# ethz-asl/voxgraph

Hardware: AMD Instinct MI355X
Metric: Mresiduals+Jacobians/s per GPU; full pose-graph solve ms (200 submaps) (higher is better)
Workload: dtype f32

## Files before the change

### voxgraph_amd/csrc/vgx_internal.h

```cpp
#ifndef VGX_INTERNAL_H_
#define VGX_INTERNAL_H_

#include <hip/hip_runtime.h>

#include <algorithm>
#include <atomic>
#include <cstdint>
#include <mutex>
#include <condition_variable>
#include <initializer_list>
#include <random>
#include <string>
#include <utility>
#include <vector>

#include "voxgraph_amd.h"

namespace vgx {


template <int VPS, int LAYOUT>
struct BrickLayout {
  static constexpr int B = VPS + 1;
  static constexpr int S = VPS / 4;
// ... 40 lines not shown
  float cos_emo, sin_emo;
  float dxs, dxc;
  float dys, dyc;
  float k1, k2;
  float pad;
};
static_assert(sizeof(PosePack) == 64, "PosePack must stay one 64-byte line");

struct alignas(16) ConstraintDev {
  GridDev grid;
  const float4* xyzd;
  const float* weight;
  const uint32_t* sample_raw;
  const double* cumulative;
  const int32_t* search_lut;
  int32_t search_buckets;
  const float4* sample_pts;
  const int32_t* inv_order;
  int64_t n_points;
  const float4* chunk_bounds;
  int64_t n;
  int64_t row0;
  int64_t prow0;
  int32_t tile_points;
  double factor;
  double no_corr_cost;
};

struct Tile {
  int32_t constraint;
  int32_t count;
  int64_t start;
};

constexpr int kMinSearchBuckets = 4096;
constexpr int kMaxSearchBuckets = 1 << 24;
constexpr int kChunkPoints = 512;
constexpr int kNormalSize = 45;
constexpr int kPartialSize = 22;

struct Context {
  int device = 0;
  hipStream_t own_stream = nullptr;
  hipStream_t stream = nullptr;
  hipEvent_t ev_start = nullptr, ev_stop = nullptr;
  std::mutex mu;
  hipStream_t tsdf_own_stream = nullptr;
  hipStream_t tsdf_stream = nullptr;
  bool stream_priorities = false;
  std::atomic<int> tsdf_integrators{0};
  hipEvent_t ev_tsdf_start = nullptr, ev_tsdf_stop = nullptr, ev_handover = nullptr;
  std::mutex tsdf_mu;
  std::mutex err_mu;
  std::string last_error;
  int cu_count = 256;
  int brick_layout = 0;
  int sampling_bricks = 1;
  struct EvalSlot {
    hipStream_t stream = nullptr;
    hipEvent_t order = nullptr;
    double* d_out = nullptr;
    int64_t out_rows = 0;
    uint32_t* d_raw = nullptr;
    uint32_t* h_raw = nullptr;
    int64_t raw_cap = 0;
    double* h_out = nullptr;
// ... 108 lines not shown
  uint32_t* d_sample_raw = nullptr;
  uint32_t* h_sample_raw = nullptr;
  std::mutex mu;
  int draw_raw(uint32_t* out);
  vgx::SamplerEngine& engine();
  bool sampling() const { return cfg.sampling_ratio != -1.0f; }
  bool points_current() const;
  vgx::ConstraintDev describe() const;
  int users = 0;
  bool destroy_requested = false;
};

struct vgx_reg_batch_s {
  vgx_ctx ctx = nullptr;
  int32_t n = 0;
  int32_t n_global = 0;
  int layout = 0;
  std::vector<vgx_reg> regs;
  std::vector<int32_t> node_pair;
  std::vector<int32_t> global_index;
  std::vector<int64_t> row_offset;
  std::vector<vgx::Tile> tiles;
  vgx::ConstraintDev* d_desc = nullptr;
  vgx::PosePack* d_pack = nullptr;
  vgx::PosePack* h_pack = nullptr;
  hipEvent_t pack_copied[2] = {nullptr, nullptr};
  int pack_turn = 0;
  vgx::Tile* d_tiles = nullptr;
  vgx::Tile* d_draw_tiles = nullptr;
  int32_t n_draw_tiles = 0;
  float4* d_drawn = nullptr;
  int32_t* d_drawn_idx = nullptr;
  unsigned char* d_tile_dead = nullptr;
  int32_t* d_tile_first = nullptr;
  double* d_partials = nullptr;
  double* d_normal = nullptr;
  double* h_normal = nullptr;
  int32_t* d_node_pair = nullptr;
  int32_t* d_global_index = nullptr;
  std::vector<vgx::Tile> reduce_tiles;
  std::vector<vgx::ConstraintDev> host_desc;
  std::vector<int32_t> host_tile_first;
  bool launch_order_made = false;
  bool launch_order_grouped = false, points_order_grouped = false;
  bool points_order_made = false;
  std::vector<int32_t> host_points_tile_first;
  vgx::Tile* d_reduce_tiles = nullptr;
  int32_t csr_nodes = 0;
  int32_t* d_node_first = nullptr;
  int32_t* d_node_items = nullptr;
  struct StreamJob {
    vgx::SamplerEngine* engine;
    int64_t offset;
    int64_t count;
  };
  std::vector<StreamJob> stream_jobs;
  uint32_t* d_raw = nullptr;
  void* d_stream_jobs = nullptr;
  bool any_sampling = false;
  bool holds_regs = false;
  double* d_rows[3] = {nullptr, nullptr, nullptr};
  char* h_rows = nullptr;
  bool rows_have[3] = {false, false, false};
  bool rows_mirrored = false;
};

namespace vgx {
#ifndef VGX_TOOLING_LIBRARY
int set_error(vgx_ctx ctx, int code, const std::string& msg);
#else
inline int set_error(vgx_ctx ctx, int code, const std::string& msg);
#endif

std::mutex& lifetime_mu();

struct DeviceBuffer {
  void* p = nullptr;
  size_t bytes = 0;
// ... 139 lines not shown
```

### voxgraph_amd/csrc/vgx_reg.hip

```cpp
#include <algorithm>
#include <cmath>
#include <cstdio>
#include <cstdlib>
#include <cstring>
#include <numeric>

#include "vgx_internal.h"

#pragma clang fp contract(off)

namespace vgx {

namespace {
struct YawQuat {
  float w, z;
};

YawQuat yaw_exp(float psi) {
  float nrm = std::sqrt(0.0f * 0.0f + 0.0f * 0.0f + psi * psi);
  double theta = (double)nrm;
  double na = theta < std::pow(2.220446049250313e-16, 0.25)
                  ? 0.5 + (theta * theta) * (1.0 / 48.0)
                  : std::sin(theta * 0.5) / theta;
  double ct = std::cos(theta * 0.5);
// ... 365 lines not shown
  }
}

__device__ __forceinline__ f32x4 sampled_point(const ConstraintDev& C, int64_t i) {
  if (C.sample_pts) return as_global(reinterpret_cast<const f32x4*>(C.sample_pts))[C.row0 + i];
  return as_global(reinterpret_cast<const f32x4*>(C.xyzd))[weighted_draw(C, i)];
}


__device__ __forceinline__ bool tile_cullable(const ConstraintDev& C) {
  return C.no_corr_cost == 0.0 && C.sample_raw == nullptr && C.chunk_bounds != nullptr;
}
template <int PPT>
__device__ __forceinline__ bool tile_outside(const ConstraintDev& C, const PosePack& P, const Tile& tile) {
  const long long chunk0 = tile.start / kChunkPoints;
  bool any_live = false;
#pragma unroll
  for (int q = 0; q < (kBlockThreads * PPT) / kChunkPoints; ++q)
    if (q * kChunkPoints < tile.count) any_live |= !chunk_outside(C.grid, P, C.chunk_bounds[chunk0 + q]);
  return !any_live;
}
template <int PPT>
__global__ __launch_bounds__(256) void reg_points_tile_dead_kernel(const ConstraintDev* __restrict__ cons,
                                                                  const PosePack* __restrict__ packs,
                                                                  const Tile* __restrict__ tiles, int n_tiles,
                                                                  unsigned char* __restrict__ dead) {
  const int t = blockIdx.x * 256 + threadIdx.x;
  if (t >= n_tiles) return;
  const Tile tile = tiles[t];
  const ConstraintDev& C = cons[tile.constraint];
  dead[t] = tile_cullable(C) && tile_outside<PPT>(C, packs[tile.constraint], tile);
}

template <int VPS, int LAYOUT, typename OUT, int PPT>
__device__ __forceinline__ void reg_eval_points_body(
    const ConstraintDev& C, const PosePack& P, const Tile& tile, int dead_hint, OUT* __restrict__ residuals,
    typename Out4<OUT>::type* __restrict__ jac_ref, typename Out4<OUT>::type* __restrict__ jac_read) {
  const GridDev g = C.grid;
  const bool sampled = C.sample_raw != nullptr;
  const bool want_jac = (jac_ref != nullptr) | (jac_read != nullptr);
  {
    bool any_live = dead_hint == 0;
    if (dead_hint < 0) {
      any_live = true;
      if (tile_cullable(C)) any_live = !tile_outside<PPT>(C, P, tile);
    }
    if (!any_live) {
#pragma unroll
      for (int j = 0; j < PPT; ++j) {
        int local = j * kBlockThreads + (int)threadIdx.x;
        if (local >= tile.count) continue;
        int64_t row = C.row0 + tile.start + local;
        store_out(&residuals[row], (OUT)0);
        if (jac_ref) store_out4(&jac_ref[row], Out4<OUT>::make(0.0, 0.0, 0.0, 0.0));
        if (jac_read) store_out4(&jac_read[row], Out4<OUT>::make(0.0, 0.0, 0.0, 0.0));
      }
      return;
    }
  }

  f32x4 pt[PPT];
  float w[PPT];
  const float* cell[PPT];
  float Dx[PPT], Dy[PPT], Dz[PPT];
  float d[PPT][8];
#pragma unroll
  for (int j = 0; j < PPT; ++j) {
    int local = j * kBlockThreads + (int)threadIdx.x;
    bool active = local < tile.count;
    int64_t i = tile.start + (active ? local : 0);
    if (sampled) {
      pt[j] = sampled_point(C, i);
      w[j] = 1.0f;
    } else {
      pt[j] = as_global(reinterpret_cast<const f32x4*>(C.xyzd))[i];
      w[j] = as_global(C.weight)[i];
    }
  }
  Located loc[PPT];
  bool have[PPT];
  const bool grid_empty = g.bricks == nullptr;
#pragma unroll
  for (int j = 0; j < PPT; ++j) {
    loc[j] = locate_stage1<VPS, LAYOUT>(g, P, pt[j].x, pt[j].y, pt[j].z);
    Dx[j] = loc[j].Dx;
    Dy[j] = loc[j].Dy;
    Dz[j] = loc[j].Dz;
    have[j] = false;
#pragma unroll
    for (int k = 0; k < 8; ++k) d[j][k] = 0.0f;
    cell[j] = nullptr;
  }
  if (!grid_empty) {
    int slot[PPT];
#pragma unroll
    for (int j = 0; j < PPT; ++j) slot[j] = as_global(g.lut)[loc[j].lut_index];
    constexpr int CELLS = BrickLayout<VPS, LAYOUT>::cells;
#pragma unroll
    for (int j = 0; j < PPT; ++j) {
      have[j] = loc[j].inside && slot[j] >= 0;
      cell[j] = g.bricks + (size_t)(have[j] ? slot[j] : 0) * CELLS + loc[j].cell_off;
    }
#pragma unroll
    for (int j = 0; j < PPT; ++j) load_neighbours<VPS, LAYOUT>(cell[j], d[j]);
  }
#pragma unroll
  for (int j = 0; j < PPT; ++j) {
    int local = j * kBlockThreads + (int)threadIdx.x;
    if (local >= tile.count) continue;
    PointEval e = eval_point(d[j], have[j], Dx[j], Dy[j], Dz[j], g.voxel_size_inv, P,
                             pt[j].x, pt[j].y, pt[j].w, w[j], C.no_corr_cost, want_jac);
    int64_t row = C.row0 + tile.start + local;
    const double f = C.factor;
    store_out(&residuals[row], (OUT)(e.r * f));
    if (jac_ref)
      store_out4(&jac_ref[row], Out4<OUT>::make((double)e.jo0 * f, (double)e.jo1 * f,
                                                (double)e.jo2 * f, (double)e.jo3 * f));
    if (jac_read)
      store_out4(&jac_read[row], Out4<OUT>::make((double)-e.jo0 * f, (double)-e.jo1 * f,
                                                 (double)-e.jo2 * f, (double)e.je3 * f));
  }
}

template <int VPS, int LAYOUT, typename OUT, int PPT>
__global__ __launch_bounds__(kBlockThreads) void reg_eval_points_kernel(
    const ConstraintDev* __restrict__ cons, const PosePack* __restrict__ packs,
    const Tile* __restrict__ tiles, const unsigned char* __restrict__ tile_dead, int n_tiles,
    OUT* __restrict__ residuals, typename Out4<OUT>::type* __restrict__ jac_ref,
    typename Out4<OUT>::type* __restrict__ jac_read, int blocked) {
  const int t = blockIdx.x;
  if (t >= n_tiles) return;
  const Tile tile = tiles[t];
  const int dead = tile_dead[t];
  const ConstraintDev& C = cons[tile.constraint];
  if (blocked) {
    using O4 = typename Out4<OUT>::type;
    constexpr long long kBlockBytes = (long long)(PPT * kBlockThreads) * (long long)(sizeof(OUT) + 2 * sizeof(O4));
    const long long first = C.row0 + tile.start;
    char* blk = reinterpret_cast<char*>(residuals) + ((C.prow0 + tile.start) / (PPT * kBlockThreads)) * kBlockBytes;
    OUT* r_t = reinterpret_cast<OUT*>(blk) - first;
    O4* jr_t = reinterpret_cast<O4*>(blk + (long long)(PPT * kBlockThreads) * (long long)sizeof(OUT)) - first;
    O4* je_t = reinterpret_cast<O4*>(blk + (long long)(PPT * kBlockThreads) * (long long)(sizeof(OUT) + sizeof(O4))) - first;
    reg_eval_points_body<VPS, LAYOUT, OUT, PPT>(C, packs[tile.constraint], tile, dead, r_t, jr_t, je_t);
    return;
  }
  reg_eval_points_body<VPS, LAYOUT, OUT, PPT>(C, packs[tile.constraint], tile, dead, residuals, jac_ref, jac_read);
}

template <int VPS, int LAYOUT, typename OUT, int PPT>
__global__ __launch_bounds__(kBlockThreads) void reg_eval_points_single_kernel(
    ConstraintDev C, PosePack P, int n_tiles, OUT* __restrict__ residuals,
    typename Out4<OUT>::type* __restrict__ jac_ref, typename Out4<OUT>::type* __restrict__ jac_read) {
  const int t = blockIdx.x;
  if (t >= n_tiles) return;
  Tile tile;
  tile.constraint = 0;
  tile.start = (int64_t)t * (kBlockThreads * PPT);
  int64_t left = C.n - tile.start;
  tile.count = (int32_t)(left < kBlockThreads * PPT ? left : kBlockThreads * PPT);
  reg_eval_points_body<VPS, LAYOUT, OUT, PPT>(C, P, tile, -1, residuals, jac_ref, jac_read);
}

constexpr int kReduceIters = 10;
constexpr int kLeanPointsPerThread = 2;
constexpr int kLeanWaves = 6;
constexpr bool kBallotSkip = true;

__device__ __forceinline__ bool eval_point_lean(const float c[8], bool have, float Dx, float Dy, float Dz,
                                                float value, float inv_f, const PosePack& P, float xi, float yi,
                                                float d_ref, float w, float u[6]) {
#pragma clang fp contract(fast)
  const float q4 = Dx * Dy, q5 = Dy * Dz, q6 = Dz * Dx;
  const float gx = q5 * c[7] + (Dz * c[6] + (Dy * c[4] + c[1]));
  const float gy = q6 * c[7] + (Dz * c[5] + (Dx * c[4] + c[2]));
  const float gz = q4 * c[7] + (Dx * c[6] + (Dy * c[5] + c[3]));
  const float val = value;
  const bool ok = have && (val == val);
  const float s = -w * inv_f;
  const float h0 = ok ? s * gx : 0.0f, h1 = ok ? s * gy : 0.0f, h2 = ok ? s * gz : 0.0f;
// ... 363 lines not shown
          }
        }
      }
      out.push_back(stream[(size_t)src][next[(size_t)src]++]);
    }
  return out;
}

static std::vector<Tile> make_draw_order(const std::vector<ConstraintDev>& desc,
                                         const std::vector<int32_t>& tile_first, const std::vector<Tile>& tiles) {
  std::vector<const void*> key;
  std::vector<std::vector<Tile>> group_tiles;
  std::vector<int64_t> group_work;
  size_t n = 0;
  for (size_t c = 0; c < desc.size(); ++c) {
    if (!desc[c].sample_raw) continue;
    size_t g = 0;
    while (g < key.size() && key[g] != (const void*)desc[c].cumulative) ++g;
    if (g == key.size()) {
      key.push_back((const void*)desc[c].cumulative);
      group_tiles.emplace_back();
      group_work.push_back(0);
    }
    for (int32_t t = tile_first[c]; t < tile_first[c + 1]; ++t) {
      group_tiles[g].push_back(tiles[(size_t)t]);
      group_work[g] += tiles[(size_t)t].count;
      ++n;
    }
  }
  return deal_to_xcds(group_tiles, group_work, n);
}

static bool make_xcd_order(const std::vector<ConstraintDev>& desc, const std::vector<int32_t>& tile_first,
                           const std::vector<int32_t>& tile_work, std::vector<Tile>& tiles, bool points_pass) {
  if (points_pass) {
    const char* e = getenv("VGX_POINTS_TILE_ORDER");
    if (e && atoi(e) == 0) return false;
  }
  const int n = (int)desc.size();
  if (n < 2 || tiles.size() < 16) return false;
  std::vector<std::vector<int>> groups;
  {
    std::vector<std::pair<const void*, int>> key;
    for (int c = 0; c < n; ++c) {
      int g = -1;
      if (!desc[(size_t)c].sample_raw)
        for (auto& k : key)
          if (k.first == (const void*)desc[(size_t)c].xyzd) g = k.second;
      if (g < 0) {
        g = (int)groups.size();
        groups.emplace_back();
        if (!desc[(size_t)c].sample_raw) key.emplace_back((const void*)desc[(size_t)c].xyzd, g);
      }
      groups[(size_t)g].push_back(c);
    }
  }
  std::vector<std::vector<Tile>> group_tiles(groups.size());
  std::vector<int64_t> group_work(groups.size(), 0);
  for (size_t g = 0; g < groups.size(); ++g) {
    int most = 0;
    for (int c : groups[g]) most = std::max(most, tile_first[(size_t)c + 1] - tile_first[(size_t)c]);
    for (int r = 0; r < most; ++r)
      for (int c : groups[g])
        if (r < tile_first[(size_t)c + 1] - tile_first[(size_t)c]) {
          const size_t t = (size_t)tile_first[(size_t)c] + (size_t)r;
          group_tiles[g].push_back(tiles[t]);
          group_work[g] += points_pass ? (int64_t)tiles[t].count * 36 + (int64_t)tile_work[t] * 52
                                       : (int64_t)tile_work[t] + 256;
        }
  }
  constexpr double kOrderShareMin = 0.3;
  constexpr double kOrderLiveMin = 0.75;
  {
    int64_t total = 0, shareable = 0;
    for (size_t g = 0; g < groups.size(); ++g) {
      int most = 0;
      for (int c : groups[g]) most = std::max(most, tile_first[(size_t)c + 1] - tile_first[(size_t)c]);
      for (int r = 0; r < most; ++r) {
        int64_t sum = 0, mx = 0;
        for (int c : groups[g])
          if (r < tile_first[(size_t)c + 1] - tile_first[(size_t)c]) {
            const int64_t w = tile_work[(size_t)tile_first[(size_t)c] + (size_t)r];
            sum += w;
            mx = std::max(mx, w);
          }
        total += sum;
        shareable += sum - mx;
      }
    }
    if (total == 0 || (double)shareable < kOrderShareMin * (double)total) return false;
    int64_t all_points = 0;
    for (const Tile& t : tiles) all_points += t.count;
    if ((double)total < kOrderLiveMin * (double)all_points) return false;
  }
  std::vector<Tile> out = deal_to_xcds(group_tiles, group_work, tiles.size());
  tiles.swap(out);
  return true;
}

__global__ __launch_bounds__(256) void reg_finalize_kernel(const ConstraintDev* __restrict__ cons,
                                                          const PosePack* __restrict__ packs,
// ... 133 lines not shown
      int item = node_items[it];
      int c = item >> 1, side = item & 1;
      const double* nb = normal + (size_t)c * kNormalSize;
      if (e < 4) {
        v += nb[1 + 4 * side + e];
      } else {
        int k = (e - 4) / 4, l = (e - 4) % 4;
        v += H(nb, 4 * side + k, 4 * side + l);
      }
    }
    double* dst = e < 4 ? &fused[1 + 4 * (int64_t)node + e]
                        : &fused[1 + 4 * (int64_t)n_nodes + 16 * (int64_t)node + (e - 4)];
    *dst = accumulate ? *dst + v : v;
  } else if (tid < n_node_elems + n_off) {
    int64_t o = tid - n_node_elems;
    int c = (int)(o / 16), e = (int)(o % 16);
    const double* nb = normal + (size_t)c * kNormalSize;
    int gidx = global_index[c];
    double* dst = &fused[1 + 20 * (int64_t)n_nodes + 16 * (int64_t)gidx + e];
    double v = H(nb, e / 4, 4 + e % 4);
    *dst = accumulate ? *dst + v : v;
  }
}

__global__ void reg_scatter_normal_kernel(const double* __restrict__ normal, int n, const int32_t* __restrict__ global_index,
                                          double* __restrict__ all) {
  const int64_t tid = (int64_t)blockIdx.x * blockDim.x + threadIdx.x;
  if (tid >= (int64_t)n * kNormalSize) return;
  const int c = (int)(tid / kNormalSize), e = (int)(tid % kNormalSize);
  all[(size_t)global_index[c] * kNormalSize + e] = normal[tid];
}

template <typename OUT>
static void launch_points(vgx_ctx ctx, int vps, int layout, const ConstraintDev* d_desc, const PosePack* d_pack,
                          const Tile* d_tiles, unsigned char* d_tile_dead, int n_tiles, void* res, void* jr,
                          void* je, bool blocked = false) {
  if (n_tiles <= 0) return;
  hipLaunchKernelGGL(reg_points_tile_dead_kernel<kPointsPerThread>, dim3((n_tiles + 255) / 256), dim3(256), 0,
                     ctx->stream, d_desc, d_pack, d_tiles, n_tiles, d_tile_dead);
  dim3 grid(((n_tiles + 7) / 8) * 8), block(kBlockThreads);
  using O4 = typename Out4<OUT>::type;
#define VGX_LAUNCH_POINTS(VPS, LAYOUT)                                                              \
  hipLaunchKernelGGL((reg_eval_points_kernel<VPS, LAYOUT, OUT, kPointsPerThread>), grid, block, 0, \
                     ctx->stream, d_desc, d_pack, d_tiles, d_tile_dead, n_tiles, (OUT*)res, (O4*)jr, (O4*)je, blocked ? 1 : 0)
  if (layout == 0) {
    if (vps == 16) VGX_LAUNCH_POINTS(16, 0);
    else VGX_LAUNCH_POINTS(8, 0);
  } else if (layout == 1) {
    if (vps == 16) VGX_LAUNCH_POINTS(16, 1);
    else VGX_LAUNCH_POINTS(8, 1);
  } else {
    if (vps == 16) VGX_LAUNCH_POINTS(16, 2);
    else VGX_LAUNCH_POINTS(8, 2);
  }
#undef VGX_LAUNCH_POINTS
}

template <typename OUT>
static void launch_points_single(hipStream_t stream, int vps, const ConstraintDev& desc, const PosePack& pack,
                                 void* res, void* jr, void* je) {
  const int n_tiles = (int)((desc.n + kTilePoints - 1) / kTilePoints);
  if (n_tiles <= 0) return;
  dim3 grid(((n_tiles + 7) / 8) * 8), block(kBlockThreads);
  using O4 = typename Out4<OUT>::type;
#define VGX_LAUNCH_SINGLE(VPS, LAYOUT)                                                                       \
  hipLaunchKernelGGL((reg_eval_points_single_kernel<VPS, LAYOUT, OUT, kPointsPerThread>), grid, block, 0, stream, \
                     desc, pack, n_tiles, (OUT*)res, (O4*)jr, (O4*)je)
  const int layout = desc.grid.layout;
  if (layout == 0) {
    if (vps == 16) VGX_LAUNCH_SINGLE(16, 0);
    else VGX_LAUNCH_SINGLE(8, 0);
  } else if (layout == 1) {
    if (vps == 16) VGX_LAUNCH_SINGLE(16, 1);
    else VGX_LAUNCH_SINGLE(8, 1);
  } else {
    if (vps == 16) VGX_LAUNCH_SINGLE(16, 2);
    else VGX_LAUNCH_SINGLE(8, 2);
// ... 555 lines not shown
    b->holds_regs = true;
  }
  *out = b;
  return VGX_OK;
}

int vgx_reg_batch_destroy(vgx_reg_batch b) {
  if (!b) return VGX_ERR_INVALID;
  (void)hipSetDevice(b->ctx->device);
  (void)hipStreamSynchronize(b->ctx->stream);
  std::vector<vgx_reg> orphans;
  if (b->holds_regs) {
    std::lock_guard<std::mutex> lt(lifetime_mu());
    for (vgx_reg r : b->regs)
      if (--r->users == 0 && r->destroy_requested) orphans.push_back(r);
  }
  for (vgx_reg r : orphans) (void)vgx_reg_destroy(r);
  for (int a = 0; a < 3; ++a)
    if (b->d_rows[a]) (void)hipFree(b->d_rows[a]);
  if (b->h_rows) (void)hipHostFree(b->h_rows);
  if (b->d_raw) (void)hipFree(b->d_raw);
  if (b->d_stream_jobs) (void)hipFree(b->d_stream_jobs);
  if (b->d_node_first) (void)hipFree(b->d_node_first);
  if (b->d_node_items) (void)hipFree(b->d_node_items);
  if (b->d_reduce_tiles) (void)hipFree(b->d_reduce_tiles);
  if (b->d_desc) (void)hipFree(b->d_desc);
  if (b->d_pack) (void)hipFree(b->d_pack);
  if (b->h_pack) (void)hipHostFree(b->h_pack);
  if (b->h_normal) (void)hipHostFree(b->h_normal);
  for (int k = 0; k < 2; ++k)
    if (b->pack_copied[k]) (void)hipEventDestroy(b->pack_copied[k]);
  if (b->d_tiles) (void)hipFree(b->d_tiles);
  if (b->d_tile_dead) (void)hipFree(b->d_tile_dead);
  if (b->d_drawn) (void)hipFree(b->d_drawn);
  if (b->d_drawn_idx) (void)hipFree(b->d_drawn_idx);
  if (b->d_draw_tiles) (void)hipFree(b->d_draw_tiles);
  if (b->d_tile_first) (void)hipFree(b->d_tile_first);
  if (b->d_partials) (void)hipFree(b->d_partials);
  if (b->d_normal) (void)hipFree(b->d_normal);
  if (b->d_node_pair) (void)hipFree(b->d_node_pair);
  if (b->d_global_index) (void)hipFree(b->d_global_index);
  delete b;
  return VGX_OK;
}

int64_t vgx_reg_batch_num_residuals(vgx_reg_batch b) { return b ? b->row_offset.back() : -1; }

int vgx_reg_batch_row_offsets(vgx_reg_batch b, int64_t* row_offset) {
  if (!b || !row_offset) return VGX_ERR_INVALID;
  std::copy(b->row_offset.begin(), b->row_offset.end(), row_offset);
  return VGX_OK;
}

static int batch_points_current(vgx_reg_batch b) {
  for (vgx_reg r : b->regs)
    if (!r->points_current())
      return set_error(b->ctx, VGX_ERR_INVALID,
                       "vgx_reg_batch: a reference submap's registration points were replaced after the "
                       "batch was created");
  return VGX_OK;
}

static int batch_begin(vgx_reg_batch b) {
  vgx_ctx ctx = b->ctx;
  int rc0 = batch_points_current(b);
  if (rc0 != VGX_OK) return rc0;
// ... 8 lines not shown
  const int per_xcd = 8 * kDrawWgsPerXcdDefault < b->n_draw_tiles ? kDrawWgsPerXcdDefault : (b->n_draw_tiles + 7) / 8;
  const dim3 grid((unsigned)(8 * per_xcd));
  hipLaunchKernelGGL(reg_draw_kernel, grid, dim3(256), 0, ctx->stream, (const ConstraintDev*)b->d_desc,
                     (const Tile*)b->d_draw_tiles, (int)b->n_draw_tiles, per_xcd, b->d_drawn_idx);
  VGX_HIP(ctx, hipGetLastError());
  hipLaunchKernelGGL(reg_gather_points_kernel, grid, dim3(256), 0, ctx->stream, (const ConstraintDev*)b->d_desc,
                     (const Tile*)b->d_draw_tiles, (int)b->n_draw_tiles, per_xcd, (const int32_t*)b->d_drawn_idx,
                     b->d_drawn);
  VGX_HIP(ctx, hipGetLastError());
  return VGX_OK;
}

static int batch_upload_packs(vgx_reg_batch b, const double* poses, int32_t n_nodes, int32_t* status) {
  vgx_ctx ctx = b->ctx;
  if (b->n == 0) return VGX_OK;
  const int turn = b->pack_turn;
  b->pack_turn ^= 1;
  VGX_HIP(ctx, hipEventSynchronize(b->pack_copied[turn]));
  PosePack* stage = b->h_pack + (size_t)turn * b->n;
  for (int c = 0; c < b->n; ++c) {
    int i = b->node_pair[2 * (size_t)c], j = b->node_pair[2 * (size_t)c + 1];
    if (i >= n_nodes || j >= n_nodes)
      return set_error(ctx, VGX_ERR_INVALID, "vgx_reg_batch: node index >= n_nodes");
    make_pose_pack(poses + 4 * (size_t)i, poses + 4 * (size_t)j, &stage[c]);
    if (status) status[c] = reg_status(b->regs[(size_t)c]);
  }
  VGX_HIP(ctx, hipMemcpyAsync(b->d_pack, stage, (size_t)b->n * sizeof(PosePack),
                              hipMemcpyHostToDevice, ctx->stream));
  VGX_HIP(ctx, hipEventRecord(b->pack_copied[turn], ctx->stream));
  return VGX_OK;
}

static int apply_launch_order(vgx_reg_batch b, const std::vector<Tile>& tiles, Tile* d_tiles,
                              const std::vector<int32_t>& tile_first, bool points_pass) {
  vgx_ctx ctx = b->ctx;
  bool& grouped = points_pass ? b->points_order_grouped : b->launch_order_grouped;
  const int n_tiles = (int)tiles.size();
  DeviceBuffer s_live;
  VGX_HIP(ctx, s_live.alloc((size_t)n_tiles * sizeof(int32_t)));
  hipLaunchKernelGGL(reg_tile_live_kernel, dim3(n_tiles), dim3(64), 0, ctx->stream, b->d_desc, b->d_pack,
                     d_tiles, n_tiles, s_live.as<int32_t>());
  VGX_HIP(ctx, hipGetLastError());
  std::vector<int32_t> work((size_t)n_tiles);
  VGX_HIP(ctx, hipMemcpyAsync(work.data(), s_live.p, work.size() * sizeof(int32_t), hipMemcpyDeviceToHost, ctx->stream));
  VGX_HIP(ctx, hipStreamSynchronize(ctx->stream));
  std::vector<Tile> ordered = tiles;
  grouped = make_xcd_order(b->host_desc, tile_first, work, ordered, points_pass);
  VGX_HIP(ctx, hipMemcpy(d_tiles, ordered.data(), ordered.size() * sizeof(Tile), hipMemcpyHostToDevice));
  return VGX_OK;
}

int vgx_reg_batch_evaluate_points(vgx_reg_batch b, const double* poses, int32_t n_nodes,
                                  void* d_residuals, void* d_jac_ref, void* d_jac_read,
                                  int32_t* status) {
  if (!b || !poses) return VGX_ERR_INVALID;
  vgx_ctx ctx = b->ctx;
  std::lock_guard<std::mutex> lk(ctx->mu);
  if (!d_residuals) return set_error(ctx, VGX_ERR_INVALID, "vgx_reg_batch_evaluate_points: residuals == NULL");
  VGX_HIP(ctx, hipSetDevice(ctx->device));
  int rc = batch_begin(b);
  if (rc == VGX_OK) rc = batch_upload_packs(b, poses, n_nodes, status);
  if (rc != VGX_OK) return rc;
  if (b->n == 0) return VGX_OK;
  if (!b->points_order_made && !b->tiles.empty()) {
    rc = apply_launch_order(b, b->tiles, b->d_tiles, b->host_points_tile_first, true);
    if (rc != VGX_OK) return rc;
    b->points_order_made = true;
  }
  launch_points<float>(ctx, b->regs[0]->reading->vps, b->layout, b->d_desc, b->d_pack, b->d_tiles, b->d_tile_dead,
                       (int)b->tiles.size(), d_residuals, d_jac_ref, d_jac_read);
  VGX_HIP(ctx, hipGetLastError());
  return VGX_OK;
}

int vgx_reg_batch_evaluate_points_f64(vgx_reg_batch b, const double* poses, int32_t n_nodes, void* d_residuals,
                                      void* d_jac_ref, void* d_jac_read, int32_t* status) {
  if (!b || !poses) return VGX_ERR_INVALID;
  vgx_ctx ctx = b->ctx;
  std::lock_guard<std::mutex> lk(ctx->mu);
  if (!d_residuals) return set_error(ctx, VGX_ERR_INVALID, "vgx_reg_batch_evaluate_points_f64: residuals == NULL");
  if (((uintptr_t)d_jac_ref | (uintptr_t)d_jac_read) & 31u)
    return set_error(ctx, VGX_ERR_INVALID, "vgx_reg_batch_evaluate_points_f64: Jacobian arrays must be 32-byte aligned (one row)");
  VGX_HIP(ctx, hipSetDevice(ctx->device));
  int rc = batch_begin(b);
  if (rc == VGX_OK) rc = batch_upload_packs(b, poses, n_nodes, status);
  if (rc != VGX_OK) return rc;
  if (b->n == 0) return VGX_OK;
  if (!b->points_order_made && !b->tiles.empty()) {
    rc = apply_launch_order(b, b->tiles, b->d_tiles, b->host_points_tile_first, true);
    if (rc != VGX_OK) return rc;
    b->points_order_made = true;
  }
  launch_points<double>(ctx, b->regs[0]->reading->vps, b->layout, b->d_desc, b->d_pack, b->d_tiles, b->d_tile_dead,
                        (int)b->tiles.size(), d_residuals, d_jac_ref, d_jac_read);
  VGX_HIP(ctx, hipGetLastError());
  return VGX_OK;
}

constexpr int64_t kRowsMirrorLimit = (int64_t)2 << 30;

int vgx_reg_batch_evaluate_rows_f64(vgx_reg_batch b, const double* poses, int32_t n_nodes, int32_t want_jac_ref,
                                    int32_t want_jac_read, int32_t* status) {
  if (!b || !poses) return VGX_ERR_INVALID;
  vgx_ctx ctx = b->ctx;
  const int64_t R = b->row_offset.back();
  {
    std::lock_guard<std::mutex> lk(ctx->mu);
    VGX_HIP(ctx, hipSetDevice(ctx->device));
    const size_t bytes[3] = {(size_t)std::max<int64_t>(R, 1) * 8, (size_t)std::max<int64_t>(R, 1) * 32, (size_t)std::max<int64_t>(R, 1) * 32};
    const bool want[3] = {true, want_jac_ref != 0, want_jac_read != 0};
    for (int a = 0; a < 3; ++a)
      if (want[a] && !b->d_rows[a] && hipMalloc(&b->d_rows[a], bytes[a]) != hipSuccess) {
        (void)hipGetLastError();
        return set_error(ctx, VGX_ERR_NOMEM, "vgx_reg_batch_evaluate_rows_f64: no device memory for the batch's own rows");
      }
    if (!b->h_rows && R > 0 && R * 72 <= kRowsMirrorLimit &&
        hipHostMalloc((void**)&b->h_rows, (size_t)R * 72, hipHostMallocDefault) != hipSuccess) {
      (void)hipGetLastError();
      b->h_rows = nullptr;
    }
    b->rows_mirrored = false;
  }
  int rc = vgx_reg_batch_evaluate_points_f64(b, poses, n_nodes, b->d_rows[0], want_jac_ref ? b->d_rows[1] : nullptr,
                                             want_jac_read ? b->d_rows[2] : nullptr, status);
  if (rc != VGX_OK) return rc;
  std::lock_guard<std::mutex> lk(ctx->mu);
  b->rows_have[0] = true;
  b->rows_have[1] = want_jac_ref != 0;
  b->rows_have[2] = want_jac_read != 0;
// ... 29 lines not shown
  if (jac_ref) VGX_HIP(ctx, hipMemcpy(jac_ref, b->d_rows[1] + 4 * r0, (size_t)n * 32, hipMemcpyDeviceToHost));
  if (jac_read) VGX_HIP(ctx, hipMemcpy(jac_read, b->d_rows[2] + 4 * r0, (size_t)n * 32, hipMemcpyDeviceToHost));
  return VGX_OK;
}

int vgx_reg_batch_blocked_layout(vgx_reg_batch b, int64_t* bytes, int32_t* rows_per_block, int64_t* first_block) {
  if (!b) return VGX_ERR_INVALID;
  if (bytes) *bytes = (int64_t)b->tiles.size() * kTilePoints * 36;
  if (rows_per_block) *rows_per_block = kTilePoints;
  if (first_block) {
    int64_t blk = 0;
    for (int c = 0; c < b->n; ++c) {
      first_block[c] = blk;
      blk += (b->regs[(size_t)c]->num_residuals + kTilePoints - 1) / kTilePoints;
    }
    first_block[b->n] = blk;
  }
  return VGX_OK;
}

int vgx_reg_batch_evaluate_points_blocked(vgx_reg_batch b, const double* poses, int32_t n_nodes, void* d_blocks,
                                          int32_t* status) {
  if (!b || !poses) return VGX_ERR_INVALID;
  vgx_ctx ctx = b->ctx;
  std::lock_guard<std::mutex> lk(ctx->mu);
  if (!d_blocks) return set_error(ctx, VGX_ERR_INVALID, "vgx_reg_batch_evaluate_points_blocked: blocks == NULL");
  if (((uintptr_t)d_blocks & 15u) != 0)
    return set_error(ctx, VGX_ERR_INVALID, "vgx_reg_batch_evaluate_points_blocked: blocks must be 16-byte aligned");
  VGX_HIP(ctx, hipSetDevice(ctx->device));
  int rc = batch_begin(b);
  if (rc == VGX_OK) rc = batch_upload_packs(b, poses, n_nodes, status);
  if (rc != VGX_OK) return rc;
  if (b->n == 0) return VGX_OK;
  if (!b->points_order_made && !b->tiles.empty()) {
    rc = apply_launch_order(b, b->tiles, b->d_tiles, b->host_points_tile_first, true);
    if (rc != VGX_OK) return rc;
    b->points_order_made = true;
  }
  launch_points<float>(ctx, b->regs[0]->reading->vps, b->layout, b->d_desc, b->d_pack, b->d_tiles, b->d_tile_dead,
                       (int)b->tiles.size(), d_blocks, d_blocks, d_blocks, true);
  VGX_HIP(ctx, hipGetLastError());
  return VGX_OK;
}

int vgx_reg_batch_choose_outputs(vgx_reg_batch b, const double* poses, int32_t n_nodes, int32_t n_candidates,
                                 void* const* d_residuals, void* const* d_jac_ref, void* const* d_jac_read, int32_t launches,
                                 int32_t chosen[3], float* ms_chosen, float* ms_trials) {
  if (!b || !poses || !d_residuals || !chosen || n_candidates <= 0 || launches <= 0) return VGX_ERR_INVALID;
  vgx_ctx ctx = b->ctx;
  if (b->any_sampling)
    return set_error(ctx, VGX_ERR_INVALID, "vgx_reg_batch_choose_outputs: a sampling batch (its trial evaluations would advance the "
                                           "sampling engines); choose the arrays with an all-points batch of the same sizes");
  for (int k = 0; k < n_candidates; ++k)
    if (!d_residuals[k] || (d_jac_ref && !d_jac_ref[k]) || (d_jac_read && !d_jac_read[k]))
      return set_error(ctx, VGX_ERR_INVALID, "vgx_reg_batch_choose_outputs: a candidate is NULL");
  hipEvent_t e0 = nullptr, e1 = nullptr;
  {
    std::lock_guard<std::mutex> lk(ctx->mu);
    VGX_HIP(ctx, hipSetDevice(ctx->device));
    if (hipEventCreate(&e0) != hipSuccess || hipEventCreate(&e1) != hipSuccess) {
      if (e0) (void)hipEventDestroy(e0);
      return set_error(ctx, VGX_ERR_HIP, "vgx_reg_batch_choose_outputs: hipEventCreate failed");
    }
  }
  int n_trials = 0;
  auto trial = [&](int i, int j, int k, float* ms) -> int {
    void* jr = d_jac_ref ? d_jac_ref[j] : nullptr;
    void* je = d_jac_read ? d_jac_read[k] : nullptr;
    int rc = vgx_reg_batch_evaluate_points(b, poses, n_nodes, d_residuals[i], jr, je, nullptr);
    if (rc != VGX_OK) return rc;
    {
      std::lock_guard<std::mutex> lk(ctx->mu);
      VGX_HIP(ctx, hipEventRecord(e0, ctx->stream));
    }
    for (int l = 0; l < launches && rc == VGX_OK; ++l)
// ... 93 lines not shown
  {
    std::lock_guard<std::mutex> lk(ctx->mu);
    (void)hipSetDevice(ctx->device);
    (void)hipStreamSynchronize(ctx->stream);
    for (int a = 0; a < 3; ++a)
      for (int k = 0; k < have; ++k)
        if (cand[a][k] && (rc != VGX_OK || k != chosen[a])) (void)hipFree(cand[a][k]);
  }
  if (rc != VGX_OK) return rc;
  *d_residuals = cand[0][chosen[0]];
  if (want[1]) *d_jac_ref = cand[1][chosen[1]];
  if (want[2]) *d_jac_read = cand[2][chosen[2]];
  return VGX_OK;
}

int vgx_reg_batch_free_outputs(vgx_reg_batch b, void* d_residuals, void* d_jac_ref, void* d_jac_read) {
  if (!b) return VGX_ERR_INVALID;
  vgx_ctx ctx = b->ctx;
  std::lock_guard<std::mutex> lk(ctx->mu);
  (void)hipSetDevice(ctx->device);
  (void)hipStreamSynchronize(ctx->stream);
  for (void* p : {d_residuals, d_jac_ref, d_jac_read})
    if (p) (void)hipFree(p);
  return VGX_OK;
}

}

template <bool COST_ONLY>
static int launch_fused_tiles(vgx_reg_batch b) {
  vgx_ctx ctx = b->ctx;
  const int n_tiles = (int)b->reduce_tiles.size();
  if (!b->launch_order_made && n_tiles > 0) {
    int rc = apply_launch_order(b, b->reduce_tiles, b->d_reduce_tiles, b->host_tile_first, false);
    if (rc != VGX_OK) return rc;
    b->launch_order_made = true;
  }
  const unsigned occupancy_pad = ctx->tsdf_integrators.load() > 0 ? 27u * 1024u : 0u;
  if (n_tiles > 0) {
    dim3 grid(n_tiles), block(kBlockThreads);
    const int vps = b->regs[0]->reading->vps;
#define VGX_LAUNCH_LEAN(VPS, LAYOUT)                                                                                \
  hipLaunchKernelGGL((reg_eval_reduce_lean_kernel<VPS, LAYOUT, COST_ONLY>), grid, block, occupancy_pad, ctx->stream, \
                     b->d_desc, b->d_pack, b->d_reduce_tiles, n_tiles, b->d_tile_first, b->d_partials)
    if (b->layout == 1) {
      if (vps == 16) VGX_LAUNCH_LEAN(16, 1);
      else VGX_LAUNCH_LEAN(8, 1);
    } else if (b->layout == 2) {
      if (vps == 16) VGX_LAUNCH_LEAN(16, 2);
      else VGX_LAUNCH_LEAN(8, 2);
    } else {
      if (vps == 16) VGX_LAUNCH_LEAN(16, 0);
      else VGX_LAUNCH_LEAN(8, 0);
    }
#undef VGX_LAUNCH_LEAN
    VGX_HIP(ctx, hipGetLastError());
  }
  return VGX_OK;
}

extern "C" {

int vgx_reg_batch_evaluate_normal(vgx_reg_batch b, const double* poses, int32_t n_nodes,
                                  void* d_normal, double* normal_host, int32_t* status) {
  if (!b || !poses) return VGX_ERR_INVALID;
  vgx_ctx ctx = b->ctx;
  std::lock_guard<std::mutex> lk(ctx->mu);
// ... 258 lines not shown
```

Before: 131,100.

## Group constraints sharing a point cloud so each block loads points once

Constraints that read the same unsampled point array are grouped into work items, each covering one tile of points and up to 32 member constraints. A new liveness kernel computes a per-item bitmask of non-culled members. The group kernel loads the tile's points once and evaluates every live member against them, writing zeros for dead members. This replaces the XCD-aware tile reordering for the points pass and trades point-load reuse for longer, serialized per-block work and possible load imbalance.

```diff
diff --git a/voxgraph_amd/csrc/vgx_internal.h b/voxgraph_amd/csrc/vgx_internal.h
--- a/voxgraph_amd/csrc/vgx_internal.h
+++ b/voxgraph_amd/csrc/vgx_internal.h
@@ -96,6 +96,15 @@
   int32_t count;
   int64_t start;
 };
+
+struct PointsItem {
+  int64_t start;
+  int32_t count;
+  int32_t member_first;
+  int32_t n_members;
+  int32_t pad;
+};
+constexpr int kMaxItemMembers = 32;
 
 constexpr int kMinSearchBuckets = 4096;
 constexpr int kMaxSearchBuckets = 1 << 24;
@@ -270,6 +279,10 @@
   float4* d_drawn = nullptr;
   int32_t* d_drawn_idx = nullptr;
   unsigned char* d_tile_dead = nullptr;
+  vgx::PointsItem* d_items = nullptr;
+  int32_t* d_item_members = nullptr;
+  uint32_t* d_item_live = nullptr;
+  int32_t n_items = 0;
   int32_t* d_tile_first = nullptr;
   double* d_partials = nullptr;
   double* d_normal = nullptr;
@@ -280,8 +293,9 @@
   std::vector<vgx::ConstraintDev> host_desc;
   std::vector<int32_t> host_tile_first;
   bool launch_order_made = false;
-  bool launch_order_grouped = false, points_order_grouped = false;
+  bool launch_order_grouped = false;
   bool points_order_made = false;
+  bool points_order_grouped = false;
   std::vector<int32_t> host_points_tile_first;
   vgx::Tile* d_reduce_tiles = nullptr;
   int32_t csr_nodes = 0;
diff --git a/voxgraph_amd/csrc/vgx_reg.hip b/voxgraph_amd/csrc/vgx_reg.hip
--- a/voxgraph_amd/csrc/vgx_reg.hip
+++ b/voxgraph_amd/csrc/vgx_reg.hip
@@ -421,38 +421,46 @@
   dead[t] = tile_cullable(C) && tile_outside<PPT>(C, packs[tile.constraint], tile);
 }
 
-template <int VPS, int LAYOUT, typename OUT, int PPT>
-__device__ __forceinline__ void reg_eval_points_body(
-    const ConstraintDev& C, const PosePack& P, const Tile& tile, int dead_hint, OUT* __restrict__ residuals,
-    typename Out4<OUT>::type* __restrict__ jac_ref, typename Out4<OUT>::type* __restrict__ jac_read) {
-  const GridDev g = C.grid;
+template <int PPT>
+__global__ __launch_bounds__(256) void reg_points_item_live_kernel(const ConstraintDev* __restrict__ cons,
+                                                                  const PosePack* __restrict__ packs,
+                                                                  const PointsItem* __restrict__ items,
+                                                                  const int32_t* __restrict__ members, int n_items,
+                                                                  uint32_t* __restrict__ item_live) {
+  const int t = blockIdx.x * 256 + threadIdx.x;
+  if (t >= n_items) return;
+  const PointsItem item = items[t];
+  Tile tile;
+  tile.start = item.start;
+  tile.count = item.count;
+  uint32_t live = 0;
+  for (int m = 0; m < item.n_members; ++m) {
+    tile.constraint = members[item.member_first + m];
+    const ConstraintDev& C = cons[tile.constraint];
+    const bool dead = tile_cullable(C) && tile_outside<PPT>(C, packs[tile.constraint], tile);
+    if (!dead) live |= 1u << m;
+  }
+  item_live[t] = live;
+}
+
+template <typename OUT, int PPT>
+__device__ __forceinline__ void write_zero_rows(const ConstraintDev& C, const Tile& tile, OUT* __restrict__ residuals,
+                                                typename Out4<OUT>::type* __restrict__ jac_ref,
+                                                typename Out4<OUT>::type* __restrict__ jac_read) {
+#pragma unroll
+  for (int j = 0; j < PPT; ++j) {
+    int local = j * kBlockThreads + (int)threadIdx.x;
+    if (local >= tile.count) continue;
+    int64_t row = C.row0 + tile.start + local;
+    store_out(&residuals[row], (OUT)0);
+    if (jac_ref) store_out4(&jac_ref[row], Out4<OUT>::make(0.0, 0.0, 0.0, 0.0));
+    if (jac_read) store_out4(&jac_read[row], Out4<OUT>::make(0.0, 0.0, 0.0, 0.0));
+  }
+}
+
+template <int PPT>
+__device__ __forceinline__ void load_tile_points(const ConstraintDev& C, const Tile& tile, f32x4 pt[PPT], float w[PPT]) {
   const bool sampled = C.sample_raw != nullptr;
-  const bool want_jac = (jac_ref != nullptr) | (jac_read != nullptr);
-  {
-    bool any_live = dead_hint == 0;
-    if (dead_hint < 0) {
-      any_live = true;
-      if (tile_cullable(C)) any_live = !tile_outside<PPT>(C, P, tile);
-    }
-    if (!any_live) {
-#pragma unroll
-      for (int j = 0; j < PPT; ++j) {
-        int local = j * kBlockThreads + (int)threadIdx.x;
-        if (local >= tile.count) continue;
-        int64_t row = C.row0 + tile.start + local;
-        store_out(&residuals[row], (OUT)0);
-        if (jac_ref) store_out4(&jac_ref[row], Out4<OUT>::make(0.0, 0.0, 0.0, 0.0));
-        if (jac_read) store_out4(&jac_read[row], Out4<OUT>::make(0.0, 0.0, 0.0, 0.0));
-      }
-      return;
-    }
-  }
-
-  f32x4 pt[PPT];
-  float w[PPT];
-  const float* cell[PPT];
-  float Dx[PPT], Dy[PPT], Dz[PPT];
-  float d[PPT][8];
 #pragma unroll
   for (int j = 0; j < PPT; ++j) {
     int local = j * kBlockThreads + (int)threadIdx.x;
@@ -466,6 +474,18 @@
       w[j] = as_global(C.weight)[i];
     }
   }
+}
+
+template <int VPS, int LAYOUT, typename OUT, int PPT>
+__device__ __forceinline__ void eval_loaded_points(
+    const ConstraintDev& C, const PosePack& P, const Tile& tile, const f32x4 pt[PPT], const float w[PPT],
+    OUT* __restrict__ residuals, typename Out4<OUT>::type* __restrict__ jac_ref,
+    typename Out4<OUT>::type* __restrict__ jac_read) {
+  const GridDev g = C.grid;
+  const bool want_jac = (jac_ref != nullptr) | (jac_read != nullptr);
+  const float* cell[PPT];
+  float Dx[PPT], Dy[PPT], Dz[PPT];
+  float d[PPT][8];
   Located loc[PPT];
   bool have[PPT];
   const bool grid_empty = g.bricks == nullptr;
@@ -511,6 +531,40 @@
   }
 }
 
+template <typename OUT, int PPT>
+__device__ __forceinline__ void rebase_to_block(const ConstraintDev& C, const Tile& tile, OUT* blocks, OUT*& r_t,
+                                                typename Out4<OUT>::type*& jr_t, typename Out4<OUT>::type*& je_t) {
+  using O4 = typename Out4<OUT>::type;
+  constexpr long long kBlockBytes = (long long)(PPT * kBlockThreads) * (long long)(sizeof(OUT) + 2 * sizeof(O4));
+  const long long first = C.row0 + tile.start;
+  char* blk = reinterpret_cast<char*>(blocks) + ((C.prow0 + tile.start) / (PPT * kBlockThreads)) * kBlockBytes;
+  r_t = reinterpret_cast<OUT*>(blk) - first;
+  jr_t = reinterpret_cast<O4*>(blk + (long long)(PPT * kBlockThreads) * (long long)sizeof(OUT)) - first;
+  je_t = reinterpret_cast<O4*>(blk + (long long)(PPT * kBlockThreads) * (long long)(sizeof(OUT) + sizeof(O4))) - first;
+}
+
+template <int VPS, int LAYOUT, typename OUT, int PPT>
+__device__ __forceinline__ void reg_eval_points_body(
+    const ConstraintDev& C, const PosePack& P, const Tile& tile, int dead_hint, OUT* __restrict__ residuals,
+    typename Out4<OUT>::type* __restrict__ jac_ref, typename Out4<OUT>::type* __restrict__ jac_read) {
+  {
+    bool any_live = dead_hint == 0;
+    if (dead_hint < 0) {
+      any_live = true;
+      if (tile_cullable(C)) any_live = !tile_outside<PPT>(C, P, tile);
+    }
+    if (!any_live) {
+      write_zero_rows<OUT, PPT>(C, tile, residuals, jac_ref, jac_read);
+      return;
+    }
+  }
+
+  f32x4 pt[PPT];
+  float w[PPT];
+  load_tile_points<PPT>(C, tile, pt, w);
+  eval_loaded_points<VPS, LAYOUT, OUT, PPT>(C, P, tile, pt, w, residuals, jac_ref, jac_read);
+}
+
 template <int VPS, int LAYOUT, typename OUT, int PPT>
 __global__ __launch_bounds__(kBlockThreads) void reg_eval_points_kernel(
     const ConstraintDev* __restrict__ cons, const PosePack* __restrict__ packs,
@@ -522,18 +576,44 @@
   const Tile tile = tiles[t];
   const int dead = tile_dead[t];
   const ConstraintDev& C = cons[tile.constraint];
-  if (blocked) {
-    using O4 = typename Out4<OUT>::type;
-    constexpr long long kBlockBytes = (long long)(PPT * kBlockThreads) * (long long)(sizeof(OUT) + 2 * sizeof(O4));
-    const long long first = C.row0 + tile.start;
-    char* blk = reinterpret_cast<char*>(residuals) + ((C.prow0 + tile.start) / (PPT * kBlockThreads)) * kBlockBytes;
-    OUT* r_t = reinterpret_cast<OUT*>(blk) - first;
-    O4* jr_t = reinterpret_cast<O4*>(blk + (long long)(PPT * kBlockThreads) * (long long)sizeof(OUT)) - first;
-    O4* je_t = reinterpret_cast<O4*>(blk + (long long)(PPT * kBlockThreads) * (long long)(sizeof(OUT) + sizeof(O4))) - first;
-    reg_eval_points_body<VPS, LAYOUT, OUT, PPT>(C, packs[tile.constraint], tile, dead, r_t, jr_t, je_t);
-    return;
-  }
-  reg_eval_points_body<VPS, LAYOUT, OUT, PPT>(C, packs[tile.constraint], tile, dead, residuals, jac_ref, jac_read);
+  OUT* r_t = residuals;
+  typename Out4<OUT>::type *jr_t = jac_ref, *je_t = jac_read;
+  if (blocked) rebase_to_block<OUT, PPT>(C, tile, residuals, r_t, jr_t, je_t);
+  reg_eval_points_body<VPS, LAYOUT, OUT, PPT>(C, packs[tile.constraint], tile, dead, r_t, jr_t, je_t);
+}
+
+template <int VPS, int LAYOUT, typename OUT, int PPT>
+__global__ __launch_bounds__(kBlockThreads) void reg_eval_points_group_kernel(
+    const ConstraintDev* __restrict__ cons, const PosePack* __restrict__ packs,
+    const PointsItem* __restrict__ items, const int32_t* __restrict__ members,
+    const uint32_t* __restrict__ item_live, int n_items, OUT* __restrict__ residuals,
+    typename Out4<OUT>::type* __restrict__ jac_ref, typename Out4<OUT>::type* __restrict__ jac_read, int blocked) {
+  const int t = blockIdx.x;
+  if (t >= n_items) return;
+  const PointsItem item = items[t];
+  const uint32_t live = item_live[t];
+  Tile tile;
+  tile.start = item.start;
+  tile.count = item.count;
+  f32x4 pt[PPT];
+  float w[PPT];
+#pragma unroll
+  for (int j = 0; j < PPT; ++j) {
+    pt[j] = f32x4{0.0f, 0.0f, 0.0f, 0.0f};
+    w[j] = 0.0f;
+  }
+  if (live) load_tile_points<PPT>(cons[members[item.member_first]], tile, pt, w);
+  for (int m = 0; m < item.n_members; ++m) {
+    tile.constraint = members[item.member_first + m];
+    const ConstraintDev& C = cons[tile.constraint];
+    OUT* r_t = residuals;
+    typename Out4<OUT>::type *jr_t = jac_ref, *je_t = jac_read;
+    if (blocked) rebase_to_block<OUT, PPT>(C, tile, residuals, r_t, jr_t, je_t);
+    if ((live >> m) & 1u)
+      eval_loaded_points<VPS, LAYOUT, OUT, PPT>(C, packs[tile.constraint], tile, pt, w, r_t, jr_t, je_t);
+    else
+      write_zero_rows<OUT, PPT>(C, tile, r_t, jr_t, je_t);
+  }
 }
 
 template <int VPS, int LAYOUT, typename OUT, int PPT>
@@ -963,11 +1043,7 @@
 }
 
 static bool make_xcd_order(const std::vector<ConstraintDev>& desc, const std::vector<int32_t>& tile_first,
-                           const std::vector<int32_t>& tile_work, std::vector<Tile>& tiles, bool points_pass) {
-  if (points_pass) {
-    const char* e = getenv("VGX_POINTS_TILE_ORDER");
-    if (e && atoi(e) == 0) return false;
-  }
+                           const std::vector<int32_t>& tile_work, std::vector<Tile>& tiles) {
   const int n = (int)desc.size();
   if (n < 2 || tiles.size() < 16) return false;
   std::vector<std::vector<int>> groups;
@@ -996,8 +1072,7 @@
         if (r < tile_first[(size_t)c + 1] - tile_first[(size_t)c]) {
           const size_t t = (size_t)tile_first[(size_t)c] + (size_t)r;
           group_tiles[g].push_back(tiles[t]);
-          group_work[g] += points_pass ? (int64_t)tiles[t].count * 36 + (int64_t)tile_work[t] * 52
-                                       : (int64_t)tile_work[t] + 256;
+          group_work[g] += (int64_t)tile_work[t] + 256;
         }
   }
   constexpr double kOrderShareMin = 0.3;
@@ -1197,17 +1272,31 @@
 }
 
 template <typename OUT>
-static void launch_points(vgx_ctx ctx, int vps, int layout, const ConstraintDev* d_desc, const PosePack* d_pack,
-                          const Tile* d_tiles, unsigned char* d_tile_dead, int n_tiles, void* res, void* jr,
-                          void* je, bool blocked = false) {
-  if (n_tiles <= 0) return;
-  hipLaunchKernelGGL(reg_points_tile_dead_kernel<kPointsPerThread>, dim3((n_tiles + 255) / 256), dim3(256), 0,
-                     ctx->stream, d_desc, d_pack, d_tiles, n_tiles, d_tile_dead);
-  dim3 grid(((n_tiles + 7) / 8) * 8), block(kBlockThreads);
+static void launch_points(vgx_reg_batch b, void* res, void* jr, void* je, bool blocked) {
+  vgx_ctx ctx = b->ctx;
+  const int vps = b->regs[0]->reading->vps, layout = b->layout;
+  const bool group = b->d_items != nullptr;
+  const int n_work = group ? (int)b->n_items : (int)b->tiles.size();
+  if (n_work <= 0) return;
+  if (group)
+    hipLaunchKernelGGL(reg_points_item_live_kernel<kPointsPerThread>, dim3((n_work + 255) / 256), dim3(256), 0, ctx->stream,
+                       b->d_desc, b->d_pack, b->d_items, b->d_item_members, n_work, b->d_item_live);
+  else
+    hipLaunchKernelGGL(reg_points_tile_dead_kernel<kPointsPerThread>, dim3((n_work + 255) / 256), dim3(256), 0, ctx->stream,
+                       b->d_desc, b->d_pack, b->d_tiles, n_work, b->d_tile_dead);
+  dim3 grid(((n_work + 7) / 8) * 8), block(kBlockThreads);
   using O4 = typename Out4<OUT>::type;
-#define VGX_LAUNCH_POINTS(VPS, LAYOUT)                                                              \
-  hipLaunchKernelGGL((reg_eval_points_kernel<VPS, LAYOUT, OUT, kPointsPerThread>), grid, block, 0, \
-                     ctx->stream, d_desc, d_pack, d_tiles, d_tile_dead, n_tiles, (OUT*)res, (O4*)jr, (O4*)je, blocked ? 1 : 0)
+#define VGX_LAUNCH_POINTS(VPS, LAYOUT)                                                                                 \
+  do {                                                                                                                 \
+    if (group)                                                                                                         \
+      hipLaunchKernelGGL((reg_eval_points_group_kernel<VPS, LAYOUT, OUT, kPointsPerThread>), grid, block, 0,           \
+                         ctx->stream, b->d_desc, b->d_pack, b->d_items, b->d_item_members, b->d_item_live, n_work,     \
+                         (OUT*)res, (O4*)jr, (O4*)je, blocked ? 1 : 0);                                                \
+    else                                                                                                               \
+      hipLaunchKernelGGL((reg_eval_points_kernel<VPS, LAYOUT, OUT, kPointsPerThread>), grid, block, 0, ctx->stream,    \
+                         b->d_desc, b->d_pack, b->d_tiles, b->d_tile_dead, n_work, (OUT*)res, (O4*)jr, (O4*)je,        \
+                         blocked ? 1 : 0);                                                                             \
+  } while (0)
   if (layout == 0) {
     if (vps == 16) VGX_LAUNCH_POINTS(16, 0);
     else VGX_LAUNCH_POINTS(8, 0);
@@ -1829,6 +1918,9 @@
     if (b->pack_copied[k]) (void)hipEventDestroy(b->pack_copied[k]);
   if (b->d_tiles) (void)hipFree(b->d_tiles);
   if (b->d_tile_dead) (void)hipFree(b->d_tile_dead);
+  if (b->d_items) (void)hipFree(b->d_items);
+  if (b->d_item_members) (void)hipFree(b->d_item_members);
+  if (b->d_item_live) (void)hipFree(b->d_item_live);
   if (b->d_drawn) (void)hipFree(b->d_drawn);
   if (b->d_drawn_idx) (void)hipFree(b->d_drawn_idx);
   if (b->d_draw_tiles) (void)hipFree(b->d_draw_tiles);
@@ -1903,9 +1995,8 @@
 }
 
 static int apply_launch_order(vgx_reg_batch b, const std::vector<Tile>& tiles, Tile* d_tiles,
-                              const std::vector<int32_t>& tile_first, bool points_pass) {
+                              const std::vector<int32_t>& tile_first) {
   vgx_ctx ctx = b->ctx;
-  bool& grouped = points_pass ? b->points_order_grouped : b->launch_order_grouped;
   const int n_tiles = (int)tiles.size();
   DeviceBuffer s_live;
   VGX_HIP(ctx, s_live.alloc((size_t)n_tiles * sizeof(int32_t)));
@@ -1916,8 +2007,70 @@
   VGX_HIP(ctx, hipMemcpyAsync(work.data(), s_live.p, work.size() * sizeof(int32_t), hipMemcpyDeviceToHost, ctx->stream));
   VGX_HIP(ctx, hipStreamSynchronize(ctx->stream));
   std::vector<Tile> ordered = tiles;
-  grouped = make_xcd_order(b->host_desc, tile_first, work, ordered, points_pass);
+  b->launch_order_grouped = make_xcd_order(b->host_desc, tile_first, work, ordered);
   VGX_HIP(ctx, hipMemcpy(d_tiles, ordered.data(), ordered.size() * sizeof(Tile), hipMemcpyHostToDevice));
+  return VGX_OK;
+}
+
+static int prepare_points_pass(vgx_reg_batch b) {
+  vgx_ctx ctx = b->ctx;
+  if (b->points_order_made || b->tiles.empty()) return VGX_OK;
+  const char* e = getenv("VGX_POINTS_TILE_ORDER");
+  if (e && atoi(e) == 0) {
+    b->points_order_grouped = false;
+    b->points_order_made = true;
+    return VGX_OK;
+  }
+  const std::vector<ConstraintDev>& desc = b->host_desc;
+  std::vector<std::vector<int32_t>> groups;
+  for (int32_t c = 0; c < b->n; ++c) {
+    const ConstraintDev& D = desc[(size_t)c];
+    if (D.n <= 0) continue;
+    size_t g = groups.size();
+    if (!D.sample_raw)
+      for (size_t k = 0; k < groups.size() && g == groups.size(); ++k) {
+        const ConstraintDev& F = desc[(size_t)groups[k][0]];
+        if (!F.sample_raw && F.xyzd == D.xyzd && F.weight == D.weight && F.n == D.n) g = k;
+      }
+    if (g == groups.size()) groups.emplace_back();
+    groups[g].push_back(c);
+  }
+  std::vector<PointsItem> items;
+  std::vector<int32_t> members;
+  bool shared = false;
+  for (const std::vector<int32_t>& grp : groups) {
+    const int32_t first = (int32_t)members.size();
+    members.insert(members.end(), grp.begin(), grp.end());
+    shared |= grp.size() > 1;
+    const int64_t n = desc[(size_t)grp[0]].n;
+    for (int64_t s = 0; s < n; s += kTilePoints)
+      for (size_t m0 = 0; m0 < grp.size(); m0 += kMaxItemMembers) {
+        PointsItem it;
+        it.start = s;
+        it.count = (int32_t)std::min<int64_t>(kTilePoints, n - s);
+        it.member_first = first + (int32_t)m0;
+        it.n_members = (int32_t)std::min<size_t>(kMaxItemMembers, grp.size() - m0);
+        it.pad = 0;
+        items.push_back(it);
+      }
+  }
+  VGX_HIP(ctx, hipMalloc((void**)&b->d_items, items.size() * sizeof(PointsItem)));
+  VGX_HIP(ctx, hipMalloc((void**)&b->d_item_members, members.size() * sizeof(int32_t)));
+  VGX_HIP(ctx, hipMalloc((void**)&b->d_item_live, items.size() * sizeof(uint32_t)));
+  VGX_HIP(ctx, hipMemcpy(b->d_items, items.data(), items.size() * sizeof(PointsItem), hipMemcpyHostToDevice));
+  VGX_HIP(ctx, hipMemcpy(b->d_item_members, members.data(), members.size() * sizeof(int32_t), hipMemcpyHostToDevice));
+  b->n_items = (int32_t)items.size();
+  b->points_order_grouped = shared;
+  b->points_order_made = true;
+  return VGX_OK;
+}
+
+static int batch_launch_points(vgx_reg_batch b, bool f64, void* res, void* jr, void* je, bool blocked = false) {
+  int rc = prepare_points_pass(b);
+  if (rc != VGX_OK) return rc;
+  if (f64) launch_points<double>(b, res, jr, je, blocked);
+  else launch_points<float>(b, res, jr, je, blocked);
+  VGX_HIP(b->ctx, hipGetLastError());
   return VGX_OK;
 }
 
@@ -1933,15 +2086,7 @@
   if (rc == VGX_OK) rc = batch_upload_packs(b, poses, n_nodes, status);
   if (rc != VGX_OK) return rc;
   if (b->n == 0) return VGX_OK;
-  if (!b->points_order_made && !b->tiles.empty()) {
-    rc = apply_launch_order(b, b->tiles, b->d_tiles, b->host_points_tile_first, true);
-    if (rc != VGX_OK) return rc;
-    b->points_order_made = true;
-  }
-  launch_points<float>(ctx, b->regs[0]->reading->vps, b->layout, b->d_desc, b->d_pack, b->d_tiles, b->d_tile_dead,
-                       (int)b->tiles.size(), d_residuals, d_jac_ref, d_jac_read);
-  VGX_HIP(ctx, hipGetLastError());
-  return VGX_OK;
+  return batch_launch_points(b, false, d_residuals, d_jac_ref, d_jac_read);
 }
 
 int vgx_reg_batch_evaluate_points_f64(vgx_reg_batch b, const double* poses, int32_t n_nodes, void* d_residuals,
@@ -1957,15 +2102,7 @@
   if (rc == VGX_OK) rc = batch_upload_packs(b, poses, n_nodes, status);
   if (rc != VGX_OK) return rc;
   if (b->n == 0) return VGX_OK;
-  if (!b->points_order_made && !b->tiles.empty()) {
-    rc = apply_launch_order(b, b->tiles, b->d_tiles, b->host_points_tile_first, true);
-    if (rc != VGX_OK) return rc;
-    b->points_order_made = true;
-  }
-  launch_points<double>(ctx, b->regs[0]->reading->vps, b->layout, b->d_desc, b->d_pack, b->d_tiles, b->d_tile_dead,
-                        (int)b->tiles.size(), d_residuals, d_jac_ref, d_jac_read);
-  VGX_HIP(ctx, hipGetLastError());
-  return VGX_OK;
+  return batch_launch_points(b, true, d_residuals, d_jac_ref, d_jac_read);
 }
 
 constexpr int64_t kRowsMirrorLimit = (int64_t)2 << 30;
@@ -2061,15 +2198,7 @@
   if (rc == VGX_OK) rc = batch_upload_packs(b, poses, n_nodes, status);
   if (rc != VGX_OK) return rc;
   if (b->n == 0) return VGX_OK;
-  if (!b->points_order_made && !b->tiles.empty()) {
-    rc = apply_launch_order(b, b->tiles, b->d_tiles, b->host_points_tile_first, true);
-    if (rc != VGX_OK) return rc;
-    b->points_order_made = true;
-  }
-  launch_points<float>(ctx, b->regs[0]->reading->vps, b->layout, b->d_desc, b->d_pack, b->d_tiles, b->d_tile_dead,
-                       (int)b->tiles.size(), d_blocks, d_blocks, d_blocks, true);
-  VGX_HIP(ctx, hipGetLastError());
-  return VGX_OK;
+  return batch_launch_points(b, false, d_blocks, d_blocks, d_blocks, true);
 }
 
 int vgx_reg_batch_choose_outputs(vgx_reg_batch b, const double* poses, int32_t n_nodes, int32_t n_candidates,
@@ -2229,7 +2358,7 @@
   vgx_ctx ctx = b->ctx;
   const int n_tiles = (int)b->reduce_tiles.size();
   if (!b->launch_order_made && n_tiles > 0) {
-    int rc = apply_launch_order(b, b->reduce_tiles, b->d_reduce_tiles, b->host_tile_first, false);
+    int rc = apply_launch_order(b, b->reduce_tiles, b->d_reduce_tiles, b->host_tile_first);
     if (rc != VGX_OK) return rc;
     b->launch_order_made = true;
   }
```

Result: slower. 128,800 (-1.8%).
